# khiner/MeshEditor

Measured on AMD Instinct MI355X. Metric: eigenpairs/sec (K/M assembly + 50-mode solve, 100k-tet mesh), higher is better.
Workload: dtype f64; 1 GPU; cube_s100k: Kuhn mesh 105456 tets / 446631 DOF, NumModes=50 NumFemModes=65, P=10 excitation points, one mesh per GPU; eigenpairs_per_mesh=65, kept_modes_per_mesh=50, parallelism=mesh-per-gpu x1

## Files before the change

### mesheditor_amd/csrc/mh_api.hip

```cpp
#include "mh_common.h"

#include <algorithm>
#include <cmath>
#include <memory>

namespace {
constexpr int TB = 256;

__global__ void k_export_blocks(const uint32_t *__restrict__ row_ptr, const uint32_t *__restrict__ col, const uint32_t *__restrict__ perm, uint32_t nnodes,
                                uint32_t *__restrict__ row_out, uint32_t *__restrict__ col_out) {
    const uint32_t r = blockIdx.x * blockDim.x + threadIdx.x;
    if (r >= nnodes) return;
    for (uint32_t p = row_ptr[r]; p < row_ptr[r + 1]; ++p) {
        row_out[p] = perm[r];
        col_out[p] = perm[col[p]];
    }
}
__global__ void k_ref_to_panel(const double *__restrict__ xref, const uint32_t *__restrict__ perm, uint32_t nnodes, uint32_t w, double *__restrict__ panel) {
    const size_t i = size_t(blockIdx.x) * blockDim.x + threadIdx.x;
    if (i >= size_t(nnodes) * 3 * w) return;
    const uint32_t c = uint32_t(i % w), comp = uint32_t((i / w) % 3), node = uint32_t(i / (size_t(3) * w));
    panel[i] = xref[size_t(c) * (size_t(3) * nnodes) + size_t(3) * perm[node] + comp];
}
template<typename S, typename D> __global__ void k_cast(const S *__restrict__ src, D *__restrict__ dst, size_t count) {
// ... 83 lines not shown
}
int mh_context_create(int device, mh_context **out) {
    if (!out) return MH_EINVAL;
    *out = nullptr;
    auto *ctx = new mh_context;
    try {
        int count = 0;
        HIP_CHECK(hipGetDeviceCount(&count));
        if (count <= 0) mh_throw(MH_EHIP, "no HIP device: libmodalhip has no CPU fallback");
        if (device < 0 || device >= count) mh_throw(MH_EINVAL, "device %d out of range (%d visible)", device, count);
        ctx->device = device;
        if (hipDeviceGetAttribute(&ctx->cu_count, hipDeviceAttributeMultiprocessorCount, device) != hipSuccess || ctx->cu_count <= 0) ctx->cu_count = 256;
        HIP_CHECK(hipSetDevice(device));
        {
            size_t free_bytes = 0, total_bytes = 0;
            if (hipMemGetInfo(&free_bytes, &total_bytes) != hipSuccess) total_bytes = 0, (void)hipGetLastError();
            ctx->pool.set_cap_for_device(total_bytes);
        }
        HIP_CHECK(hipStreamCreateWithFlags(&ctx->stream, hipStreamNonBlocking));
        ROCBLAS_CHECK(rocblas_create_handle(&ctx->blas));
        ROCBLAS_CHECK(rocblas_set_stream(ctx->blas, ctx->stream));
        ROCBLAS_CHECK(rocblas_set_pointer_mode(ctx->blas, rocblas_pointer_mode_host));
        ROCBLAS_CHECK(rocblas_set_atomics_mode(ctx->blas, rocblas_atomics_not_allowed));
        *out = ctx;
        return MH_OK;
    } catch (const std::exception &e) {
        const int code = mh_guard(ctx, e);
        fprintf(stderr, "modalhip: %s\n", e.what());
        if (ctx->blas) rocblas_destroy_handle(ctx->blas);
        if (ctx->blas_aux) rocblas_destroy_handle(ctx->blas_aux);
        if (ctx->aux_stream) (void)hipStreamDestroy(ctx->aux_stream);
        if (ctx->aux2_stream) (void)hipStreamDestroy(ctx->aux2_stream);
        for (hipEvent_t ev : ctx->ahead_ev) (void)hipEventDestroy(ev);
        if (ctx->stream) (void)hipStreamDestroy(ctx->stream);
        delete ctx;
        return code;
    }
}
void mh_context_destroy(mh_context *ctx) {
    if (!ctx) return;
    (void)hipSetDevice(ctx->device);
    (void)hipStreamSynchronize(ctx->stream);
    if (ctx->blas) rocblas_destroy_handle(ctx->blas);
    if (ctx->blas_aux) rocblas_destroy_handle(ctx->blas_aux);
    if (ctx->aux_stream) (void)hipStreamDestroy(ctx->aux_stream);
    if (ctx->aux2_stream) (void)hipStreamDestroy(ctx->aux2_stream);
    for (hipEvent_t e : ctx->ahead_ev) (void)hipEventDestroy(e);
    if (ctx->stream) (void)hipStreamDestroy(ctx->stream);
    delete ctx;
}
const char *mh_last_error(const mh_context *ctx) { return ctx ? ctx->last_error.c_str() : "null context"; }
int mh_context_synchronize(mh_context *ctx) {
    if (!ctx) return MH_EINVAL;
    try {
        HIP_CHECK(hipStreamSynchronize(ctx->stream));
        return MH_OK;
    } catch (const std::exception &e) { return mh_guard(ctx, e); }
}
void *mh_context_stream(mh_context *ctx) { return ctx ? ctx->stream : nullptr; }
int mh_context_time_kernels(mh_context *ctx, int enable) {
    if (!ctx) return MH_EINVAL;
    try {
        mh_timer_flush(ctx);
        ctx->time_kernels = enable != 0;
        for (auto &t : ctx->totals) t = {};
        return MH_OK;
    } catch (const std::exception &e) { return mh_guard(ctx, e); }
}
int mh_context_kernel_class_stats(mh_context *ctx, int kernel_class, uint64_t *launches, double *total_ms, double *total_work) {
    if (!ctx || kernel_class < 0 || kernel_class >= MH_KERNEL_CLASSES) return MH_EINVAL;
    try {
        mh_timer_flush(ctx);
        const auto &t = ctx->totals[kernel_class];
        if (launches) *launches = t.launches;
        if (total_ms) *total_ms = t.ms;
// ... 205 lines not shown
```

### mesheditor_amd/csrc/mh_common.h

```cpp
#pragma once
#include "../../include/modalhip.h"

#include <hip/hip_runtime.h>
#include <rocblas/rocblas.h>
#include <rocsolver/rocsolver.h>

#include <algorithm>
#include <cstdarg>
#include <cstdio>
#include <cstdlib>
#include <cstring>
#include <iterator>
#include <limits>
#include <map>
#include <mutex>
#include <stdexcept>
#include <string>
#include <vector>

struct MhError : std::runtime_error {
    int code;
    MhError(int c, const std::string &m) : std::runtime_error(m), code(c) {}
};

// ... 207 lines not shown
    }
    ~DevicePool() {
        trim();
        for (auto &kv : live) (void)hipFree(kv.first);
    }
};

struct mh_context {
    int device{0};
    int cu_count{256};
    hipStream_t stream{nullptr};
    hipStream_t aux_stream{nullptr};
    bool aux_stream_ready() {
        if (!aux_stream && hipStreamCreateWithFlags(&aux_stream, hipStreamNonBlocking) != hipSuccess) aux_stream = nullptr;
        if (aux_stream && !blas_aux) {
            if (rocblas_create_handle(&blas_aux) != rocblas_status_success) blas_aux = nullptr;
            else if (rocblas_set_stream(blas_aux, aux_stream) != rocblas_status_success) {
                (void)rocblas_destroy_handle(blas_aux);
                blas_aux = nullptr;
            }
        }
        return aux_stream != nullptr && blas_aux != nullptr;
    }
    hipStream_t aux2_stream{nullptr};
    std::vector<hipEvent_t> ahead_ev;
    bool aux2_stream_ready(size_t events = 0) {
        if (!aux2_stream && hipStreamCreateWithFlags(&aux2_stream, hipStreamNonBlocking) != hipSuccess) aux2_stream = nullptr, (void)hipGetLastError();
        while (aux2_stream && ahead_ev.size() < events) {
            hipEvent_t e = nullptr;
            if (hipEventCreateWithFlags(&e, hipEventDisableTiming) != hipSuccess) { (void)hipGetLastError(); return false; }
            ahead_ev.push_back(e);
        }
        return aux2_stream != nullptr;
    }
    rocblas_handle blas{nullptr};
    rocblas_handle blas_aux{nullptr};
    DevicePool pool;
    std::string last_error;
    hipEvent_t ev0{nullptr}, ev1{nullptr};
    void *gram_ws{nullptr};
    size_t gram_ws_bytes{0};
    uint32_t *iota{nullptr};
    unsigned long long *sytrd_xch{nullptr};
    uint32_t sytrd_epoch{0};
    int *sytrd_flag{nullptr};
    unsigned long long *sytrd_xch_wide{nullptr};
    uint32_t sytrd_epoch_wide{0};
    bool exchange_disabled{false};
    uint32_t sytrd_redos{0};
    unsigned long long *rr_check{nullptr};
    struct MhRrTrace *rr_trace{nullptr};
    bool time_kernels{false};
    std::vector<std::pair<hipEvent_t, hipEvent_t>> timer_events;
    std::vector<double> timer_work;
    std::vector<int> timer_class;
    size_t timer_used{0};
    struct ClassTotals {
        double ms{0}, work{0};
        uint64_t launches{0};
    } totals[MH_KERNEL_CLASSES];
};
void mh_timer_flush(mh_context *ctx);
struct TimedLaunch {
    mh_context *ctx;
    bool on;
    size_t slot{0};
// ... 248 lines not shown
```

### mesheditor_amd/csrc/mh_eigs.hip

```cpp
#include "mh_common.h"

#include <algorithm>
#include <cmath>
#include <memory>
#include <condition_variable>
#include <mutex>
#include <numeric>
#include <optional>
#include <type_traits>

__global__ void k_shift_values(const double *kval, const double *mval, size_t nblocks, double sigma, double *aval);
__global__ void k_diag_inverse(const uint32_t *row_ptr, const uint32_t *col, const double *aval, uint32_t nnodes, double *dinv);
__global__ void k_coarse_matrix(const uint32_t *row_ptr, const uint32_t *col, const double *aval, const double *tmat, const uint32_t *agg_of, const uint32_t *agg_ptr,
                                const uint32_t *agg_nodes, uint32_t nagg, double *a0);
__global__ void k_fix_coarse_diag(double *a0, uint32_t n0, double rel);

namespace {
constexpr int TB = 256;

std::mutex g_solve_mutex;
struct Switches {
    bool verbose = getenv("MH_VERBOSE") != nullptr;
    bool fp32_prec = !(getenv("MH_PRECOND_FP64") && atoi(getenv("MH_PRECOND_FP64")) != 0);
    int deg2 = 0, deg1 = 0, gamma = 0;
    double cheb_ratio = 0.0, cheb_ratio1 = 0.0;
    bool test_sytrd_giveup = getenv("MH_TEST") && strstr(getenv("MH_TEST"), "sytrd_giveup");
    bool no_tridiag_wide = getenv("MH_TEST") && strstr(getenv("MH_TEST"), "no_tridiag_wide");
    bool test_last_resort = getenv("MH_TEST") && strstr(getenv("MH_TEST"), "last_resort");
    bool test_coarse_pivot = getenv("MH_TEST") && strstr(getenv("MH_TEST"), "coarse_pivot");
    bool test_selfcheck_fail = getenv("MH_TEST") && strstr(getenv("MH_TEST"), "selfcheck_fail");
    bool lmax_low = getenv("MH_TEST") && strstr(getenv("MH_TEST"), "lmax_low");
    bool potrf_chain = getenv("MH_TEST") && strstr(getenv("MH_TEST"), "potrf_chain");
    bool no_poly_start = getenv("MH_TEST") && strstr(getenv("MH_TEST"), "no_poly_start");
    Switches() {
        if (const char *c = getenv("MH_CYCLE")) {
            double v[5] = {0, 0, 0, 0, 0};
            sscanf(c, "%lf,%lf,%lf,%lf,%lf", &v[0], &v[1], &v[2], &v[3], &v[4]);
            deg2 = std::max(0, int(v[0])), deg1 = std::max(0, int(v[1])), gamma = std::max(0, int(v[2]));
            cheb_ratio = v[3];
            cheb_ratio1 = v[4];
        }
    }
};
const Switches &switches() {
    static const Switches s;
    return s;
}
constexpr int kPowerIterations = 20;
constexpr uint32_t kPrecondColumns = 256;
constexpr uint32_t kSkipP = 4;
constexpr uint32_t kGuardPercent = 10;
constexpr float kFlatShape = 1e-4f;
constexpr size_t kDenseLastResort = 12288;
constexpr int kLastResortCg = 8;

struct PhaseLock {
    std::mutex m;
    std::condition_variable cv;
    int readers = 0, writers_waiting = 0;
    bool writer = false;
    void lock_shared() {
        std::unique_lock<std::mutex> l(m);
        cv.wait(l, [&] { return !writer && writers_waiting == 0; });
        ++readers;
    }
    void unlock_shared() {
        std::unique_lock<std::mutex> l(m);
        if (--readers == 0) cv.notify_all();
    }
    void lock() {
        std::unique_lock<std::mutex> l(m);
        ++writers_waiting;
        cv.wait(l, [&] { return !writer && readers == 0; });
        --writers_waiting;
        writer = true;
    }
    void unlock() {
        std::unique_lock<std::mutex> l(m);
        writer = false;
        cv.notify_all();
    }
};
constexpr int kMaxDevices = 64;
PhaseLock g_phase_of_device[kMaxDevices];
PhaseLock &phase_of(int device) { return g_phase_of_device[unsigned(device) % kMaxDevices]; }
const bool g_concurrent = !(getenv("MH_CONCURRENT_SOLVES") && atoi(getenv("MH_CONCURRENT_SOLVES")) == 0);
struct SharedPhase {
    PhaseLock &phase;
    bool held = false, enabled = true;
    explicit SharedPhase(int device, bool on = true) : phase(phase_of(device)), enabled(on) { acquire(); }
    ~SharedPhase() { release(); }
    void acquire() { if (g_concurrent && enabled && !held) { phase.lock_shared(); held = true; } }
    void release() { if (held) { phase.unlock_shared(); held = false; } }
};
struct ExclusivePhase {
    PhaseLock &phase;
    bool held = false;
    explicit ExclusivePhase(int device) : phase(phase_of(device)) {
        if (g_concurrent) {
            phase.lock();
            held = true;
            (void)hipSetDevice(device);
            (void)hipDeviceSynchronize();
        }
    }
    ~ExclusivePhase() { if (held) phase.unlock(); }
};

struct Timer {
    mh_context *ctx;
    hipEvent_t a, b;
    explicit Timer(mh_context *c) : ctx(c) {
        HIP_CHECK(hipEventCreate(&a));
        HIP_CHECK(hipEventCreate(&b));
        HIP_CHECK(hipEventRecord(a, ctx->stream));
    }
    double stop() {
        HIP_CHECK(hipEventRecord(b, ctx->stream));
        HIP_CHECK(hipEventSynchronize(b));
// ... 1128 lines not shown
        const uint32_t nb = uint32_t(div_up(n, rpb));
        k_coldot_partial<<<dim3(nb, div_up(w, 64)), 64, 0, ctx->stream>>>(u, v, n, w, scratch, rpb);
        KERNEL_CHECK();
        k_colsumsq_final<<<w, 256, 0, ctx->stream>>>(scratch, nb, w, out);
        KERNEL_CHECK();
    }
    template<typename Prec> void solve(Prec &prec, const double *r, double *z, uint32_t w, int iters) {
        hipStream_t st = ctx->stream;
        HIP_CHECK(hipMemsetAsync(z, 0, n * w * sizeof(double), st));
        HIP_CHECK(hipMemcpyAsync(rr.get(), r, n * w * sizeof(double), hipMemcpyDeviceToDevice, st));
        prec.apply(rr, zz, w);
        HIP_CHECK(hipMemcpyAsync(p.get(), zz.get(), n * w * sizeof(double), hipMemcpyDeviceToDevice, st));
        dot(rr, zz, rz, w);
        for (int k = 0; k < iters; ++k) {
            mh_spmm(ctx, sys->L2, sys->L2.aval, p, ap, nullptr, nullptr, w);
            dot(p, ap, pap, w);
            k_cg_advance<<<grid1(n * w), TB, 0, st>>>(z, rr, p, ap, rz, pap, n * w, w);
            KERNEL_CHECK();
            if (k + 1 == iters) break;
            prec.apply(rr, zz, w);
            dot(rr, zz, rz_new, w);
            k_cg_direction<<<grid1(n * w), TB, 0, st>>>(p, zz, rz_new, rz, n * w, w);
            KERNEL_CHECK();
            HIP_CHECK(hipMemcpyAsync(rz.get(), rz_new.get(), w * sizeof(double), hipMemcpyDeviceToDevice, st));
        }
    }
};
}

namespace {
struct BlockLobpcg {
    mh_system *sys;
    mh_context *ctx;
    hipStream_t st;
    const size_t n;
    const uint32_t nev, b, mmax;
    const double sigma, residual_tol;
    const uint32_t max_iters;
    const float *seed_basis;
    const uint32_t seed_rows, seed_cols;
    const volatile unsigned char *cancel;
    volatile float *progress;
    mh_profile &prof;
    mh_profile *profile;
    SharedPhase iterating;
    Timer t_iter;
    double precond_seconds = 0;
    double best_worst_active = 1e300;
    int floor_strikes = 0;
    std::vector<double> hist_active;
    uint32_t pairs_at_floor = 0;
    DevArray<double> X, AX, MX, Xn, AXn, MXn, W, AW, MW, P, MP, Pn, MPn, R, Rw;
    DevArray<double> gA, gM, gM0, gA0, App, evals, ework, Cp, T1, H, H2, G, dscale, Linv, theta_d, rn_d, mn_d, scratch, Ct, norms_d, theta_act_d, Hp, Up, Vp, T1p;
    DevArray<double> Linv_p, T1p2;
    DevArray<uint32_t> idx_d, pos_d;
    DevArray<double> Rr, res_partial, res_blocks, res_norms_d;
    std::vector<double> rr_evals;
    std::vector<uint32_t> res_act, res_pos;
    std::vector<double> res_norms;
    uint32_t res_pitch = 0;
    bool res_ready = false, rw_from_rr = false;
    DevArray<int> info;
    int inner_cg = 0;
    std::unique_ptr<Precond<float>> prec32;
    std::unique_ptr<Precond<double>> prec64;
    std::unique_ptr<PanelCg> panel_cg;
    const bool verbose = switches().verbose, fp32_prec = switches().fp32_prec;
    const bool pproj_ok;
    const bool scaled_norms;
    bool warm = false;
    bool w_implicit = false;
    int last_spread = 1 << 20;
    bool p_needs_explicit = false;
    uint32_t wp = 0;
    uint32_t iters = 0, nconv = 0, redos_at_start = 0;
    bool poly_allowed = true;
    std::vector<double> theta, rn, mn, xn, norms, theta_act, hist_worst;
    double anorm = 0;
    std::vector<uint32_t> act, order, hist_nconv;
    std::vector<uint8_t> locked;
    bool converged = false;
    bool gm_identity = false;
    bool p_implicit = false;
    bool lazy_images = false;
    uint32_t w = 0, wa = 0, m = 0, wp_new = 0;

    BlockLobpcg(mh_system *system, uint32_t nev_, uint32_t block, double sigma_, double residual_tol_, uint32_t max_iters_, const float *seed_basis_, uint32_t seed_rows_,
                uint32_t seed_cols_, const volatile unsigned char *cancel_, volatile float *progress_, mh_profile &prof_, mh_profile *profile_, int inner_cg_ = 0)
        : sys(system), ctx(system->ctx), st(system->ctx->stream), n(size_t(3) * system->n_nodes), nev(nev_), b(block), mmax(3 * block), sigma(sigma_), residual_tol(residual_tol_),
          max_iters(max_iters_), seed_basis(seed_basis_), seed_rows(seed_rows_), seed_cols(seed_cols_), cancel(cancel_), progress(progress_), prof(prof_), profile(profile_),
          iterating(system->ctx->device, true), t_iter(system->ctx), pproj_ok(block <= 128), scaled_norms(system->patches2.any()), theta(block), rn(block), mn(block), xn(block), norms(3 * size_t(block)),
          theta_act(block), order(block), locked(block, 0) {
        inner_cg = inner_cg_;
        for (DevArray<double> *panel : {&X, &AX, &MX, &Xn, &AXn, &MXn, &W, &AW, &MW, &P, &Pn, &R, &Rw}) panel->reset(ctx, n * b);
        if (!pproj_ok)
            for (DevArray<double> *panel : {&MP, &MPn}) panel->reset(ctx, n * b);
        for (DevArray<double> *small : {&gA, &gM, &gM0, &gA0}) small->reset(ctx, size_t(mmax) * mmax);
        for (DevArray<double> *small : {&App, &H, &H2, &Linv, &Hp, &Up, &Vp, &T1p}) small->reset(ctx, size_t(b) * b);
        Linv_p.reset(ctx, size_t(b) * b);
        T1p2.reset(ctx, size_t(mmax) * b);
        for (DevArray<double> *small : {&Cp, &T1}) small->reset(ctx, size_t(mmax) * b);
        for (DevArray<double> *small : {&evals, &ework}) small->reset(ctx, mmax);
        for (DevArray<double> *small : {&dscale, &theta_d, &rn_d, &mn_d, &theta_act_d}) small->reset(ctx, b);
        G.reset(ctx, size_t(b) * 2 * b);
        Ct.reset(ctx, size_t(mmax) * 2 * b);
        norms_d.reset(ctx, 3 * size_t(b));
        idx_d.reset(ctx, b);
        pos_d.reset(ctx, b);
        if (b <= 128) {
            const uint32_t pmax = (b + 1u) & ~1u;
            Rr.reset(ctx, n * pmax);
            res_partial.reset(ctx, size_t(2) * sys->n_nodes * pmax);
            res_blocks.reset(ctx, size_t(div_up(sys->n_nodes, 48)) * 2 * pmax);
            res_norms_d.reset(ctx, size_t(2) * pmax);
            res_norms.resize(size_t(2) * pmax);
        }
        info.reset(ctx, 2);
        if (fp32_prec && !(sys->worst_quality < kFlatShape) && !inner_cg) prec32 = std::make_unique<Precond<float>>(sys, std::min(b, kPrecondColumns));
        else prec64 = std::make_unique<Precond<double>>(sys, std::min(b, kPrecondColumns));
        if (inner_cg) panel_cg = std::make_unique<PanelCg>(sys, std::min(b, kPrecondColumns));
        auto hd = sys->L2.dinv.to_host();
        double dmin = 1e300;
        for (double v : hd) dmin = std::min(dmin, v);
        anorm = sys->L2.lmax / dmin;
    }


    bool chol_orthonormalise(double *V, double *MV, double *AV, uint32_t w, bool transform_images = true, bool allow_implicit = false,
                             const double *hp = nullptr, uint32_t hp_rows = 0) {
        gram(ctx, n, V, w, MV, w, G, w);
        if (hp) {
            const double minus = -1, plus = 1;
            small_dgemm(ctx, rocblas_operation_transpose, rocblas_operation_none, rocblas_int(w), rocblas_int(w), rocblas_int(hp_rows), &minus, hp,
                                        rocblas_int(hp_rows), hp, rocblas_int(hp_rows), &plus, G, rocblas_int(w));
        }
        k_scale_gram<<<grid1(size_t(w) * w), TB, 0, st>>>(G, w, w, dscale);
        KERNEL_CHECK();
        double *Gs = G.get() + size_t(w) * w;
        int hinfo = 0;
        bool fused_inverse = false;
        {
            last_spread = 1 << 20;
            if (w <= 128) {
                fused_inverse = !switches().potrf_chain;
                if (fused_inverse) mh_potrf_small_inverse(ctx, Gs, w, info, dscale, Linv);
                else mh_potrf_small(ctx, Gs, w, info);
                int both[2] = {0, 0};
                info.download(both, 2);
                hinfo = both[0];
                last_spread = both[1];
            } else {
                mh_potrf(ctx, Gs, w, w, info);
                info.download(&hinfo, 1);
            }
        }
        p_needs_explicit = false;
        if (hp && (hinfo != 0 || last_spread >= 16 * 8)) {
            p_needs_explicit = true;
            return true;
        }
        if (hinfo != 0) return false;
        if (!fused_inverse) {
            k_unscale_chol<<<grid1(size_t(w) * w), TB, 0, st>>>(Gs, w, w, dscale);
            KERNEL_CHECK();
        }
        if (w > 256) {
            panel_trsm(ctx, n, V, w, Gs, w);
            if (MV) panel_trsm(ctx, n, MV, w, Gs, w);
            if (AV) panel_trsm(ctx, n, AV, w, Gs, w);
        } else {
            if (!fused_inverse) {
                HIP_CHECK(hipMemsetAsync(Linv, 0, size_t(w) * w * sizeof(double), st));
                ROCBLAS_CHECK(rocblas_dtrtri(ctx->blas, rocblas_fill_lower, rocblas_diagonal_non_unit, w, Gs, w, Linv, w));
            }
            w_implicit = allow_implicit && !transform_images && last_spread < 16 * 8;
            if (!w_implicit) mh_combine(ctx, n, V, w, nullptr, 0, nullptr, 0, Linv, w, V, w, nullptr);
            if (MV && transform_images) mh_combine(ctx, n, MV, w, nullptr, 0, nullptr, 0, Linv, w, MV, w, nullptr);
            if (AV && transform_images) mh_combine(ctx, n, AV, w, nullptr, 0, nullptr, 0, Linv, w, AV, w, nullptr);
        }
        return true;
    }

    void precondition(const double *r, double *z, uint32_t w) {
        precondition_in_slabs(ctx, n, r, z, w, [&](const double *rp, double *zp, uint32_t wc) {
            if (panel_cg) panel_cg->solve(*prec64, rp, zp, wc, inner_cg);
            else if (prec32) prec32->apply(rp, zp, wc);
            else prec64->apply(rp, zp, wc);
        });
    }

    void start() {
        redos_at_start = ctx->sytrd_redos;
        if (ctx->rr_check) HIP_CHECK(hipMemsetAsync(ctx->rr_check, 0, sizeof(unsigned long long), st));
        k_random_panel<<<grid1(n * b), TB, 0, st>>>(X, n * b, 20260710ull);
        KERNEL_CHECK();
        warm = seed_basis && seed_rows == n && seed_cols >= nev;
        if (warm) {
            const uint32_t ncols = std::min(seed_cols, b);
            DevArray<float> seed(ctx, n * ncols);
            seed.upload(seed_basis, n * ncols);
            k_load_seed<<<grid1(n * ncols), TB, 0, st>>>(seed, sys->perm, sys->n_nodes, ncols, b, X);
            KERNEL_CHECK();
            HIP_CHECK(hipStreamSynchronize(st));
        }
        const uint32_t n_rigid = 6 * sys->n_components;
        const bool seed_rigid = b >= n_rigid + 6;
        if (!seed_rigid && sys->n_components > 1)
            mh_throw(MH_EINVAL, "the mesh consists of %u disconnected bodies (%u zero modes): more than a block of %u columns can seed", sys->n_components, n_rigid, b);
        const auto inject_rigid_modes = [&] {
            k_inject_rbm<<<grid1(sys->n_nodes), TB, 0, st>>>(sys->node_xyz, sys->node_component, sys->component_centroid, sys->n_components, sys->n_nodes, X, b, 0);
            KERNEL_CHECK();
        };
        if (seed_rigid) inject_rigid_modes();
// ... 44 lines not shown
            if (with_poly) {
                if (verbose) fprintf(stderr, "[lobpcg] polynomial start block rank deficient: random block instead\n");
                poly_allowed = false;
                start();
                return;
            }
            mh_throw(MH_ENOTCONVERGED, "initial block is rank deficient");
        }
        mh_spmm(ctx, sys->L2, sys->L2.aval, X, AX, sys->L2.mval, MX, b);
        {
            gram(ctx, n, X, b, AX, b, gA, b);
            gram(ctx, n, X, b, MX, b, gM, b);
            const int hinfo = mh_rr_solve(ctx, gA, gM, b, evals, ework, info);
            if (hinfo != 0) mh_throw(MH_ENOTCONVERGED, "initial Rayleigh-Ritz failed (info %d)", hinfo);
            panel_mul(ctx, n, X, b, gA, b, Xn, b, 1.0, 0.0);
            panel_mul(ctx, n, AX, b, gA, b, AXn, b, 1.0, 0.0);
            panel_mul(ctx, n, MX, b, gA, b, MXn, b, 1.0, 0.0);
            std::swap(X, Xn); std::swap(AX, AXn); std::swap(MX, MXn);
            evals.download(theta.data(), b);
        }
    }

    bool converged_or_locked(uint32_t it) {
        if (cancel && *cancel) mh_throw(MH_ECANCELLED, "cancelled");
        if (g_concurrent) {
            iterating.release();
            iterating.acquire();
        }
        bool fused = res_ready;
        if (fused)
            for (const uint32_t i : res_act) fused = fused && !(std::abs(theta[i]) < 10.0 * std::abs(sigma));
        res_ready = false;
        rw_from_rr = fused;
        if (fused) {
            res_norms_d.download(res_norms.data(), size_t(2) * res_pitch);
            for (size_t k = 0; k < res_act.size(); ++k) {
                rn[res_act[k]] = res_norms[k];
                mn[res_act[k]] = res_norms[res_pitch + k];
            }
        } else {
        theta_d.upload(theta.data(), b);
        {
            const uint32_t rpb = 256, nblk = div_up(n, rpb);
            if (scratch.count < size_t(nblk) * 3 * b) scratch.reset(ctx, size_t(nblk) * 3 * b);
            dim3 grid(nblk, div_up(b, 64));
            k_residual_norms<<<grid, 64, 0, st>>>(AX, MX, X, theta_d, 10.0 * std::abs(sigma), R, n, b, rpb, scratch, scaled_norms ? sys->L2.dinv.get() : nullptr);
            KERNEL_CHECK();
            k_colsumsq_final<<<3 * b, 256, 0, st>>>(scratch, nblk, 3 * b, norms_d);
            KERNEL_CHECK();
            norms_d.download(norms.data(), 3 * size_t(b));
            std::copy(norms.begin(), norms.begin() + b, rn.begin());
            std::copy(norms.begin() + b, norms.begin() + 2 * b, mn.begin());
            std::copy(norms.begin() + 2 * b, norms.end(), xn.begin());
        }
        }
        act.clear();
        for (uint32_t i = 0; i < b; ++i) {
            const double rel = std::sqrt(rn[i]) / (std::abs(theta[i]) * std::sqrt(mn[i]));
            const bool near_shift = std::abs(theta[i]) < 10.0 * std::abs(sigma);
            const double floor_norm = scaled_norms ? sys->L2.lmax * std::sqrt(xn[i]) : anorm * std::sqrt(xn[i]);
            const double floor_factor = it == 0 && !warm && sys->worst_quality < kFlatShape ? 65536.0 : 256.0;
            const bool ok = rel < residual_tol || (near_shift && std::sqrt(rn[i]) < floor_factor * 2.2e-16 * floor_norm);
            if (ok) locked[i] = 1;
            if (!locked[i]) act.push_back(i);
        }
        std::iota(order.begin(), order.end(), 0u);
        std::stable_sort(order.begin(), order.end(), [&](uint32_t a, uint32_t c) { return theta[a] < theta[c]; });
        nconv = 0;
// ... 48 lines not shown
    void search_directions(uint32_t it) {
        w = uint32_t(act.size());
        idx_d.upload(act.data(), w);
        const double *residuals = Rw.get();
        if (rw_from_rr) {
            if (act == res_act && res_pitch == w) {
                residuals = Rr.get();
            } else {
                std::vector<uint32_t> &pos = res_pos;
                pos.assign(w, 0);
                size_t q = 0;
                for (uint32_t k = 0; k < w; ++k) {
                    while (q < res_act.size() && res_act[q] != act[k]) ++q;
                    if (q == res_act.size()) mh_throw(MH_EHIP, "active column %u was not active before", act[k]);
                    pos[k] = uint32_t(q);
                }
                pos_d.upload(pos.data(), w);
                k_gather_cols<<<grid1(n * w), TB, 0, st>>>(Rr, pos_d, Rw, n, res_pitch, w);
                KERNEL_CHECK();
            }
        } else {
            k_gather_cols<<<grid1(n * w), TB, 0, st>>>(R, idx_d, Rw, n, b, w);
            KERNEL_CHECK();
        }
        for (uint32_t k = 0; k < w; ++k) theta_act[k] = theta[act[k]];
        theta_act_d.upload(theta_act.data(), w);
        {
            Timer tp(ctx);
            precondition(residuals, W, w);
            precond_seconds += tp.stop();
            prof.op_applications += w;
        }
        bool ok = true;
        p_implicit = false;
        if (pproj_ok && wp) {
            gram(ctx, n, MX, b, W, w, H, b);
            mh_pack_stacked(ctx, H, b, nullptr, 0, w, -1.0, Ct);
            mh_combine(ctx, n, X, b, nullptr, 0, nullptr, 0, Ct, w, W, w, nullptr, true);
            mh_spmm(ctx, sys->L2, sys->L2.aval, W, AW, sys->L2.mval, MW, w);
            gram(ctx, n, P, wp, MW, w, Hp, wp);
            lazy_images = true;
            w_implicit = false;
            ok = chol_orthonormalise(W, MW, AW, w, false, true, Hp, wp);
            if (!ok) mh_throw(MH_ENOTCONVERGED, "search directions lost rank at iteration %u", it);
            if (p_needs_explicit) {
                mh_pack_stacked(ctx, Hp, wp, nullptr, 0, w, -1.0, Ct);
                mh_combine(ctx, n, P, wp, nullptr, 0, nullptr, 0, Ct, w, W, w, nullptr, true);
                mh_spmm(ctx, sys->L2, sys->L2.aval, W, AW, sys->L2.mval, MW, w);
                lazy_images = w <= 256;
                ok = chol_orthonormalise(W, MW, AW, w, !lazy_images, lazy_images);
                if (!ok) mh_throw(MH_ENOTCONVERGED, "search directions lost rank at iteration %u", it);
            } else {
                p_implicit = true;
            }
        } else {
            gram(ctx, n, MX, b, W, w, H, b);
            if (wp) gram(ctx, n, MP, wp, W, w, H2, wp);
            mh_pack_stacked(ctx, H, b, H2, wp, w, -1.0, Ct);
            mh_combine(ctx, n, X, b, P, wp, nullptr, 0, Ct, w, W, w, nullptr, true);
            mh_spmm(ctx, sys->L2, sys->L2.aval, W, AW, sys->L2.mval, MW, w);
            lazy_images = w <= 256;
            w_implicit = false;
            ok = chol_orthonormalise(W, MW, AW, w, !lazy_images, lazy_images);
            if (!ok) mh_throw(MH_ENOTCONVERGED, "search directions lost rank at iteration %u", it);
        }
    }

    void rayleigh_ritz(uint32_t it) {
        wa = w;
        m = wa + w + wp;
        for (int attempt = 0; attempt < 2; ++attempt) {
            HIP_CHECK(hipMemsetAsync(gA, 0, size_t(m) * m * sizeof(double), st));
            HIP_CHECK(hipMemsetAsync(gM, 0, size_t(m) * m * sizeof(double), st));
            k_set_identity_blocks<<<grid1(wa), TB, 0, st>>>(gA, gM, theta_act_d, wa, m);
            KERNEL_CHECK();
            const double unit_one = 1;
            auto left_corrected = [&](double *block, uint32_t cols) {
                if (w_implicit)
                    ROCBLAS_CHECK(rocblas_dtrmm(ctx->blas, rocblas_side_left, rocblas_fill_lower, rocblas_operation_none, rocblas_diagonal_non_unit, rocblas_int(w),
                                                rocblas_int(cols), &unit_one, Linv, rocblas_int(w), block, rocblas_int(m), block, rocblas_int(m)));
            };
            mh_gram(ctx, n, W, w, AX, wa, gA.get() + wa, m, b, idx_d);
            left_corrected(gA.get() + wa, wa);
            const double unit = 1;
            auto untransformed = [&](double *block, uint32_t rows) {
                if (lazy_images)
                    ROCBLAS_CHECK(rocblas_dtrmm(ctx->blas, rocblas_side_right, rocblas_fill_lower, rocblas_operation_transpose, rocblas_diagonal_non_unit, rocblas_int(rows),
                                                rocblas_int(w), &unit, Linv, rocblas_int(w), block, rocblas_int(m), block, rocblas_int(m)));
            };
            gram(ctx, n, W, w, AW, w, gA.get() + size_t(wa) * m + wa, m);
            if (p_implicit && wp) {
                const double plus = 1, nil = 0;
                double *bw = gA.get() + size_t(wa) * m + wa, *bp = gA.get() + size_t(wa) * m + wa + w;
                gram(ctx, n, P, wp, AW, w, bp, m);
                small_dgemm(ctx, rocblas_operation_transpose, rocblas_operation_none, rocblas_int(w), rocblas_int(w), rocblas_int(wp), &plus, Hp, rocblas_int(wp), bp,
                                            rocblas_int(m), &nil, Up, rocblas_int(w));
                small_dgemm(ctx, rocblas_operation_none, rocblas_operation_none, rocblas_int(wp), rocblas_int(w), rocblas_int(wp), &plus, App, rocblas_int(wp), Hp,
                                            rocblas_int(wp), &nil, T1p, rocblas_int(wp));
                small_dgemm(ctx, rocblas_operation_transpose, rocblas_operation_none, rocblas_int(w), rocblas_int(w), rocblas_int(wp), &plus, Hp, rocblas_int(wp), T1p,
                                            rocblas_int(wp), &nil, Vp, rocblas_int(w));
                k_sub_block<<<grid1(size_t(wp) * w), TB, 0, st>>>(bp, m, T1p, wp, wp, w);
                k_wblock_fix<<<grid1(size_t(w) * w), TB, 0, st>>>(bw, m, Up, Vp, w);
                KERNEL_CHECK();
            }
            untransformed(gA.get() + size_t(wa) * m + wa, w);
            left_corrected(gA.get() + size_t(wa) * m + wa, w);
            const bool w_block_trusted = last_spread < 16 * 8 && !(p_implicit && wp == 0);
            gm_identity = w_block_trusted;
            if (w_block_trusted) {
                k_place_block<<<grid1(size_t(w) * w), TB, 0, st>>>(gM.get() + size_t(wa) * m + wa, m, nullptr, w);
                KERNEL_CHECK();
            } else {
                gram(ctx, n, W, w, MW, w, gM.get() + size_t(wa) * m + wa, m);
                untransformed(gM.get() + size_t(wa) * m + wa, w);
            }
            if (verbose) fprintf(stderr, "[lobpcg] it %3u Cholesky-QR diagonal spread 2^%.1f%s\n", it, last_spread / 16.0, w_block_trusted ? "" : " (W block measured)");
            if (wp) {
                if (!p_implicit) gram(ctx, n, P, wp, AW, w, gA.get() + size_t(wa) * m + wa + w, m);
                untransformed(gA.get() + size_t(wa) * m + wa + w, wp);
                {
                    k_place_block<<<grid1(size_t(wp) * wp), TB, 0, st>>>(gA.get() + size_t(wa + w) * m + wa + w, m, App, wp);
                    k_place_block<<<grid1(size_t(wp) * wp), TB, 0, st>>>(gM.get() + size_t(wa + w) * m + wa + w, m, nullptr, wp);
                    KERNEL_CHECK();
                }
            }
            k_symmetrize_lower<<<grid1(size_t(m) * m), TB, 0, st>>>(gA, m, m);
            KERNEL_CHECK();
            HIP_CHECK(hipMemcpyAsync(gA0, gA, size_t(m) * m * sizeof(double), hipMemcpyDeviceToDevice, st));
            HIP_CHECK(hipMemcpyAsync(gM0, gM, size_t(m) * m * sizeof(double), hipMemcpyDeviceToDevice, st));
            rr_evals.clear();
            const int hinfo = mh_rr_solve(ctx, gA, gM, m, evals, ework, info, wa, gm_identity, &rr_evals);
            if (hinfo == 0) break;
            if (attempt == 1 || wp == 0) mh_throw(MH_ENOTCONVERGED, "Rayleigh-Ritz failed at iteration %u (info %d)", it, hinfo);
            wp = 0;
            m = wa + w;
        }
        if (rr_evals.size() == wa) std::copy(rr_evals.begin(), rr_evals.end(), theta_act.begin());
        else evals.download(theta_act.data(), wa);
        for (uint32_t k = 0; k < wa; ++k) theta[act[k]] = theta_act[k];
    }

    void conjugate_directions(uint32_t it) {
        const double one = 1, zero = 0, mone = -1;
        wp_new = w;
        k_build_cp<<<grid1(size_t(m) * w), TB, 0, st>>>(gA, nullptr, wa, m, w, m, Cp, m);
        KERNEL_CHECK();
        const double *mcp = gm_identity ? Cp.get() : T1.get();
        if (!gm_identity) ROCBLAS_CHECK(rocblas_dsymm(ctx->blas, rocblas_side_left, rocblas_fill_lower, m, w, &one, gM0, m, Cp, m, &zero, T1, m));
        small_dgemm(ctx, rocblas_operation_transpose, rocblas_operation_none, wa, w, m, &one, gA, m, mcp, m, &zero, H, wa);
        small_dgemm(ctx, rocblas_operation_none, rocblas_operation_none, m, w, wa, &mone, gA, m, H, wa, &one, Cp, m);
        if (!gm_identity) ROCBLAS_CHECK(rocblas_dsymm(ctx->blas, rocblas_side_left, rocblas_fill_lower, m, w, &one, gM0, m, Cp, m, &zero, T1, m));
        small_dgemm(ctx, rocblas_operation_transpose, rocblas_operation_none, w, w, m, &one, Cp, m, mcp, m, &zero, G, w);
        k_scale_gram<<<grid1(size_t(w) * w), TB, 0, st>>>(G, w, w, dscale);
        KERNEL_CHECK();
        {
            double *Gs = G.get() + size_t(w) * w;
            int hinfo = 0;
            const bool fused = w <= 128 && !switches().potrf_chain;
            {
                if (fused) mh_potrf_small_inverse(ctx, Gs, w, info, dscale, Linv_p);
                else mh_potrf(ctx, Gs, w, w, info);
                info.download(&hinfo, 1);
            }
            if (hinfo != 0) {
                wp_new = 0;
            } else if (fused) {
                mh_small_gemm(ctx, false, true, m, w, w, 1.0, Cp, m, Linv_p, w, 0.0, T1p2, m);
                HIP_CHECK(hipMemcpyAsync(Cp, T1p2, size_t(m) * w * sizeof(double), hipMemcpyDeviceToDevice, st));
            } else {
                k_unscale_chol<<<grid1(size_t(w) * w), TB, 0, st>>>(Gs, w, w, dscale);
                KERNEL_CHECK();
                ROCBLAS_CHECK(rocblas_dtrsm(ctx->blas, rocblas_side_right, rocblas_fill_lower, rocblas_operation_transpose, rocblas_diagonal_non_unit, m, w, &one, Gs, w, Cp, m));
            }
        }
        if (!warm && it < kSkipP && !hist_worst.empty() && hist_worst.back() > 0.5) wp_new = 0;
        if (wp_new) {
            small_dgemm(ctx, rocblas_operation_none, rocblas_operation_none, m, wp_new, m, &one, gA0, m, Cp, m, &zero, T1, m);
            small_dgemm(ctx, rocblas_operation_transpose, rocblas_operation_none, wp_new, wp_new, m, &one, Cp, m, T1, m, &zero, App, wp_new);
        }
    }

    void update_basis(uint32_t it) {
        mh_pack_coefficients(ctx, gA, wa, Cp, wp_new, m, m, Ct);
        {
            const uint32_t pitch = (wa + 1u) & ~1u;
            if (w_implicit) {
                const double unit = 1;
                double *rows = Ct.get() + size_t(wa) * (wa + wp_new);
                ROCBLAS_CHECK(rocblas_dtrmm(ctx->blas, rocblas_side_right, rocblas_fill_lower, rocblas_operation_none, rocblas_diagonal_non_unit, rocblas_int(wa + wp_new),
                                            rocblas_int(w), &unit, Linv, rocblas_int(w), rows, rocblas_int(wa + wp_new), rows, rocblas_int(wa + wp_new)));
            }
            if (p_implicit && wp) {
                const double minus = -1, plus = 1;
                const rocblas_int pitchc = rocblas_int(wa + wp_new);
                double *rows_w = Ct.get() + size_t(wa) * (wa + wp_new), *rows_p = Ct.get() + size_t(wa + w) * (wa + wp_new);
                ROCBLAS_CHECK(rocblas_dgemm(ctx->blas, rocblas_operation_none, rocblas_operation_transpose, pitchc, rocblas_int(wp), rocblas_int(w), &minus, rows_w, pitchc, Hp,
                                            rocblas_int(wp), &plus, rows_p, pitchc));
            }
            mh_combine(ctx, n, X, wa, W, w, P, wp, Ct, wa + wp_new, Xn, wa, Pn, false, b, idx_d, pitch);
            if (wp_new && !pproj_ok) mh_spmm(ctx, sys->L2, nullptr, Pn, nullptr, sys->L2.mval, MPn, wp_new);
            if (pitch == wa) k_scatter_cols<<<grid1(n * wa), TB, 0, st>>>(Xn.get(), idx_d, X.get(), n, b, wa);
            else k_scatter_cols_pitch<<<grid1(n * wa), TB, 0, st>>>(Xn.get(), pitch, idx_d, X.get(), n, b, wa);
            KERNEL_CHECK();
            if (Rr.count) {
                mh_spmm_mapped(ctx, sys->L2, sys->L2.aval, Xn, AX, sys->L2.mval, MX, pitch, b, wa, idx_d, evals, Rr, res_partial, scaled_norms ? sys->L2.dinv.get() : nullptr);
                const uint32_t rpb = 48, nblk = div_up(sys->n_nodes, rpb), w2 = 2 * pitch;
                dim3 grid(nblk, div_up(w2, 64));
                k_colsum_partial<<<grid, 64, 0, st>>>(res_partial, sys->n_nodes, w2, res_blocks, rpb);
                KERNEL_CHECK();
                k_colsumsq_final<<<w2, 256, 0, st>>>(res_blocks, nblk, w2, res_norms_d);
                KERNEL_CHECK();
                res_act = act;
                res_pitch = pitch;
                res_ready = true;
            } else {
                mh_spmm_mapped(ctx, sys->L2, sys->L2.aval, Xn, AX, sys->L2.mval, MX, pitch, b, wa, idx_d);
            }
        }
        std::swap(P, Pn); std::swap(MP, MPn);
        wp = wp_new;
    }

    void finish(double *eigenvalues) {
        prof.restarts = iters;
        prof.op_solve = precond_seconds;
        if (!converged) mh_throw(MH_ENOTCONVERGED, "LOBPCG: %u of %u pairs converged in %u iterations", nconv, nev, iters);
        for (uint32_t k = 0; k < nev; ++k) eigenvalues[k] = theta[order[k]] + sigma;
        sys->plain_residual = -1.0;
        if (scaled_norms) {
            theta_d.upload(theta.data(), b);
            const uint32_t rpb = 256, nblk = div_up(n, rpb);
            if (scratch.count < size_t(nblk) * 3 * b) scratch.reset(ctx, size_t(nblk) * 3 * b);
            k_residual_norms<<<dim3(nblk, div_up(b, 64)), 64, 0, st>>>(AX, MX, X, theta_d, 10.0 * std::abs(sigma), R, n, b, rpb, scratch, nullptr);
            KERNEL_CHECK();
            k_colsumsq_final<<<3 * b, 256, 0, st>>>(scratch, nblk, 3 * b, norms_d);
            KERNEL_CHECK();
            norms_d.download(norms.data(), 3 * size_t(b));
            double worst = 0;
            for (uint32_t k = 0; k < nev; ++k) {
                const uint32_t i = order[k];
                if (std::abs(theta[i]) < 10.0 * std::abs(sigma)) continue;
                worst = std::max(worst, std::sqrt(norms[i]) / (std::abs(theta[i]) * std::sqrt(norms[b + i])));
            }
            sys->plain_residual = worst;
            if (verbose) fprintf(stderr, "[lobpcg] accepted in the Jacobi-scaled norm at %.1e; worst elastic pair in the plain 2-norm: %.2e\n", residual_tol, worst);
        }
        sys->evecs.reset(ctx, n * nev);
        sys->evec_cols = nev;
        idx_d.upload(order.data(), nev);
        k_gather_cols<<<grid1(n * nev), TB, 0, st>>>(X, idx_d, sys->evecs, n, b, nev);
        KERNEL_CHECK();
        HIP_CHECK(hipStreamSynchronize(st));
        prof.iterate = t_iter.stop();
        read_health();
        sys->profile = prof;
        if (profile) *profile = prof;
        if (switches().test_selfcheck_fail && !ctx->exchange_disabled) prof.rr_selfcheck = 1.0;
        if (!(prof.rr_selfcheck < 1e-6))
            mh_throw(MH_EHIP, "Rayleigh-Ritz self-check failed: a step's eigenpairs leave a relative residual of %.2e against the step's own matrix", prof.rr_selfcheck);
    }
    void read_health() {
        prof.sytrd_redos = ctx->sytrd_redos - redos_at_start;
        prof.pairs_at_floor = pairs_at_floor;
        prof.rr_selfcheck = 0.0;
        if (ctx->rr_check) {
            unsigned long long bits = 0;
            HIP_CHECK(hipMemcpyAsync(&bits, ctx->rr_check, sizeof(bits), hipMemcpyDeviceToHost, st));
            HIP_CHECK(hipStreamSynchronize(st));
            memcpy(&prof.rr_selfcheck, &bits, sizeof(double));
        }
    }

    void run(double *eigenvalues) {
        start();
        for (uint32_t it = 0; it <= max_iters; ++it) {
            if (converged_or_locked(it)) break;
            search_directions(it);
            rayleigh_ritz(it);
            conjugate_directions(it);
            update_basis(it);
        }
        finish(eigenvalues);
    }
};
struct Attempt {
    mh_system *sys;
    uint32_t nev, b;
    double sigma, residual_tol;
    const float *seed;
    uint32_t srows, scols;
    const volatile unsigned char *cancel;
    volatile float *progress;
    double *eigenvalues;
    mh_profile &prof;
    mh_profile *profile;
    std::optional<MhError> run(uint32_t max_iters, int inner_cg = 0) {
        try {
            BlockLobpcg solver(sys, nev, b, sigma, residual_tol, max_iters, seed, srows, scols, cancel, progress, prof, profile, inner_cg);
            solver.run(eigenvalues);
            return std::nullopt;
        } catch (const MhError &e) {
            return e;
        }
    }
    void reset_profile() {
        prof = sys->profile;
        prof.dofs = uint32_t(size_t(3) * sys->n_nodes);
    }
// ... 211 lines not shown
```

Measured before the change: 614.2 eigenpairs/s.

## Overlap small Cholesky factor with Gram products and defer column scatter behind norm readback

In LOBPCG's search-direction orthonormalisation, the small Gram scaling and Cholesky/inverse now run on the aux stream. The Rayleigh-Ritz Gram products (W'AX, W'AW, P'AW) are queued on the main stream while the host waits on the factor's info readback, and Rayleigh-Ritz reuses them when the implicit path holds. Residual norms are copied into pinned host memory with an event, and the column scatter is queued after that copy, so the next iteration's host wait does not cover the scatter kernel. This removes host-sync bubbles at the cost of extra events, stream switching inside the context, and speculative Gram work that is thrown away when the factor turns out ill-conditioned.

```diff
diff --git a/mesheditor_amd/csrc/mh_api.hip b/mesheditor_amd/csrc/mh_api.hip
--- a/mesheditor_amd/csrc/mh_api.hip
+++ b/mesheditor_amd/csrc/mh_api.hip
@@ -139,6 +139,7 @@
         if (ctx->aux_stream) (void)hipStreamDestroy(ctx->aux_stream);
         if (ctx->aux2_stream) (void)hipStreamDestroy(ctx->aux2_stream);
         for (hipEvent_t ev : ctx->ahead_ev) (void)hipEventDestroy(ev);
+        ctx->chain_release();
         if (ctx->stream) (void)hipStreamDestroy(ctx->stream);
         delete ctx;
         return code;
@@ -148,6 +149,8 @@
     if (!ctx) return;
     (void)hipSetDevice(ctx->device);
     (void)hipStreamSynchronize(ctx->stream);
+    if (ctx->aux_stream) (void)hipStreamSynchronize(ctx->aux_stream);
+    ctx->chain_release();
     if (ctx->blas) rocblas_destroy_handle(ctx->blas);
     if (ctx->blas_aux) rocblas_destroy_handle(ctx->blas_aux);
     if (ctx->aux_stream) (void)hipStreamDestroy(ctx->aux_stream);
diff --git a/mesheditor_amd/csrc/mh_common.h b/mesheditor_amd/csrc/mh_common.h
--- a/mesheditor_amd/csrc/mh_common.h
+++ b/mesheditor_amd/csrc/mh_common.h
@@ -263,6 +263,27 @@
             ahead_ev.push_back(e);
         }
         return aux2_stream != nullptr;
+    }
+    struct ChainReport {
+        int w[2];
+        double norms[2 * 128];
+    };
+    enum { kChainFork = 0, kChainW, kChainNorms, kChainEvents };
+    hipEvent_t chain_ev[kChainEvents]{};
+    ChainReport *chain_host{nullptr};
+    bool chain_ready() {
+        if (!chain_host && hipHostMalloc(reinterpret_cast<void **>(&chain_host), sizeof(ChainReport), hipHostMallocDefault) != hipSuccess) chain_host = nullptr, (void)hipGetLastError();
+        for (hipEvent_t &e : chain_ev)
+            if (!e && hipEventCreateWithFlags(&e, hipEventDisableTiming) != hipSuccess) { e = nullptr; (void)hipGetLastError(); return false; }
+        return chain_host != nullptr;
+    }
+    void chain_release() {
+        for (hipEvent_t &e : chain_ev) {
+            if (e) (void)hipEventDestroy(e);
+            e = nullptr;
+        }
+        if (chain_host) (void)hipHostFree(chain_host);
+        chain_host = nullptr;
     }
     rocblas_handle blas{nullptr};
     rocblas_handle blas_aux{nullptr};
diff --git a/mesheditor_amd/csrc/mh_eigs.hip b/mesheditor_amd/csrc/mh_eigs.hip
--- a/mesheditor_amd/csrc/mh_eigs.hip
+++ b/mesheditor_amd/csrc/mh_eigs.hip
@@ -1,7 +1,9 @@
 #include "mh_common.h"
 
 #include <algorithm>
+#include <atomic>
 #include <cmath>
+#include <functional>
 #include <memory>
 #include <condition_variable>
 #include <mutex>
@@ -32,6 +34,9 @@
     bool lmax_low = getenv("MH_TEST") && strstr(getenv("MH_TEST"), "lmax_low");
     bool potrf_chain = getenv("MH_TEST") && strstr(getenv("MH_TEST"), "potrf_chain");
     bool no_poly_start = getenv("MH_TEST") && strstr(getenv("MH_TEST"), "no_poly_start");
+    bool serial_chains = getenv("MH_TEST") && strstr(getenv("MH_TEST"), "serial_chains");
+    bool w_report_ill = getenv("MH_TEST") && strstr(getenv("MH_TEST"), "w_report_ill");
+    bool cp_report_fail = getenv("MH_TEST") && strstr(getenv("MH_TEST"), "cp_report_fail");
     Switches() {
         if (const char *c = getenv("MH_CYCLE")) {
             double v[5] = {0, 0, 0, 0, 0};
@@ -49,6 +54,7 @@
 constexpr int kPowerIterations = 20;
 constexpr uint32_t kPrecondColumns = 256;
 constexpr uint32_t kSkipP = 4;
+constexpr uint32_t kHookIteration = 6;
 constexpr uint32_t kGuardPercent = 10;
 constexpr float kFlatShape = 1e-4f;
 constexpr size_t kDenseLastResort = 12288;
@@ -85,6 +91,13 @@
 PhaseLock g_phase_of_device[kMaxDevices];
 PhaseLock &phase_of(int device) { return g_phase_of_device[unsigned(device) % kMaxDevices]; }
 const bool g_concurrent = !(getenv("MH_CONCURRENT_SOLVES") && atoi(getenv("MH_CONCURRENT_SOLVES")) == 0);
+std::atomic<int> g_iterating_on_device[kMaxDevices];
+struct IteratingOnDevice {
+    std::atomic<int> &count;
+    explicit IteratingOnDevice(int device) : count(g_iterating_on_device[unsigned(device) % kMaxDevices]) { count.fetch_add(1); }
+    ~IteratingOnDevice() { count.fetch_sub(1); }
+    bool alone() const { return count.load() == 1; }
+};
 struct SharedPhase {
     PhaseLock &phase;
     bool held = false, enabled = true;
@@ -1279,6 +1292,7 @@
 struct BlockLobpcg {
     mh_system *sys;
     mh_context *ctx;
+    IteratingOnDevice in_flight{ctx->device};
     hipStream_t st;
     const size_t n;
     const uint32_t nev, b, mmax;
@@ -1331,6 +1345,12 @@
     bool p_implicit = false;
     bool lazy_images = false;
     uint32_t w = 0, wa = 0, m = 0, wp_new = 0;
+    bool overlap = false, overlap_side = false;
+    bool can_overlap = false, can_side = false;
+    bool raw_grams_queued = false;
+    bool norms_in_flight = false;
+    uint32_t cur_it = 0;
+    bool hook_w_fired = false, hook_cp_fired = false;
 
     BlockLobpcg(mh_system *system, uint32_t nev_, uint32_t block, double sigma_, double residual_tol_, uint32_t max_iters_, const float *seed_basis_, uint32_t seed_rows_,
                 uint32_t seed_cols_, const volatile unsigned char *cancel_, volatile float *progress_, mh_profile &prof_, mh_profile *profile_, int inner_cg_ = 0)
@@ -1363,6 +1383,8 @@
             res_norms.resize(size_t(2) * pmax);
         }
         info.reset(ctx, 2);
+        can_overlap = pproj_ok && !switches().serial_chains && !switches().potrf_chain && ctx->chain_ready();
+        can_side = can_overlap && ctx->aux_stream_ready();
         if (fp32_prec && !(sys->worst_quality < kFlatShape) && !inner_cg) prec32 = std::make_unique<Precond<float>>(sys, std::min(b, kPrecondColumns));
         else prec64 = std::make_unique<Precond<double>>(sys, std::min(b, kPrecondColumns));
         if (inner_cg) panel_cg = std::make_unique<PanelCg>(sys, std::min(b, kPrecondColumns));
@@ -1372,23 +1394,36 @@
         anorm = sys->L2.lmax / dmin;
     }
 
+    ~BlockLobpcg() {
+        if (can_side) (void)hipStreamSynchronize(ctx->aux_stream);
+    }
+
 
     bool chol_orthonormalise(double *V, double *MV, double *AV, uint32_t w, bool transform_images = true, bool allow_implicit = false,
-                             const double *hp = nullptr, uint32_t hp_rows = 0) {
+                             const double *hp = nullptr, uint32_t hp_rows = 0, const std::function<void()> *beside = nullptr) {
         gram(ctx, n, V, w, MV, w, G, w);
         if (hp) {
             const double minus = -1, plus = 1;
             small_dgemm(ctx, rocblas_operation_transpose, rocblas_operation_none, rocblas_int(w), rocblas_int(w), rocblas_int(hp_rows), &minus, hp,
                                         rocblas_int(hp_rows), hp, rocblas_int(hp_rows), &plus, G, rocblas_int(w));
         }
-        k_scale_gram<<<grid1(size_t(w) * w), TB, 0, st>>>(G, w, w, dscale);
-        KERNEL_CHECK();
         double *Gs = G.get() + size_t(w) * w;
         int hinfo = 0;
         bool fused_inverse = false;
+        const bool side_by_side = beside && overlap_side && w <= 128;
+        if (!side_by_side) {
+            k_scale_gram<<<grid1(size_t(w) * w), TB, 0, st>>>(G, w, w, dscale);
+            KERNEL_CHECK();
+        }
         {
             last_spread = 1 << 20;
-            if (w <= 128) {
+            if (side_by_side) {
+                fused_inverse = true;
+                int both[2] = {0, 0};
+                factor_beside(w, *beside, both);
+                hinfo = both[0];
+                last_spread = both[1];
+            } else if (w <= 128) {
                 fused_inverse = !switches().potrf_chain;
                 if (fused_inverse) mh_potrf_small_inverse(ctx, Gs, w, info, dscale, Linv);
                 else mh_potrf_small(ctx, Gs, w, info);
@@ -1401,6 +1436,11 @@
                 info.download(&hinfo, 1);
             }
         }
+        if (switches().w_report_ill && allow_implicit && !hook_w_fired && cur_it >= kHookIteration) {
+            hook_w_fired = true;
+            last_spread = 16 * 8;
+            if (verbose) fprintf(stderr, "[lobpcg] it %3u MH_TEST=w_report_ill: the factor's report reads ill-conditioned%s\n", cur_it, side_by_side ? " (Gram products were queued beside it)" : "");
+        }
         p_needs_explicit = false;
         if (hp && (hinfo != 0 || last_spread >= 16 * 8)) {
             p_needs_explicit = true;
@@ -1426,6 +1466,30 @@
             if (AV && transform_images) mh_combine(ctx, n, AV, w, nullptr, 0, nullptr, 0, Linv, w, AV, w, nullptr);
         }
         return true;
+    }
+
+    void factor_beside(uint32_t w, const std::function<void()> &beside, int both[2]) {
+        hipStream_t aux = ctx->aux_stream;
+        double *Gs = G.get() + size_t(w) * w;
+        HIP_CHECK(hipEventRecord(ctx->chain_ev[mh_context::kChainFork], st));
+        HIP_CHECK(hipStreamWaitEvent(aux, ctx->chain_ev[mh_context::kChainFork], 0));
+        k_scale_gram<<<grid1(size_t(w) * w), TB, 0, aux>>>(G, w, w, dscale);
+        KERNEL_CHECK();
+        ctx->stream = aux;
+        try {
+            mh_potrf_small_inverse(ctx, Gs, w, info, dscale, Linv);
+        } catch (...) {
+            ctx->stream = st;
+            throw;
+        }
+        ctx->stream = st;
+        HIP_CHECK(hipMemcpyAsync(ctx->chain_host->w, info.get(), 2 * sizeof(int), hipMemcpyDeviceToHost, aux));
+        HIP_CHECK(hipEventRecord(ctx->chain_ev[mh_context::kChainW], aux));
+        beside();
+        HIP_CHECK(hipEventSynchronize(ctx->chain_ev[mh_context::kChainW]));
+        both[0] = ctx->chain_host->w[0];
+        both[1] = ctx->chain_host->w[1];
+        HIP_CHECK(hipStreamWaitEvent(st, ctx->chain_ev[mh_context::kChainW], 0));
     }
 
     void precondition(const double *r, double *z, uint32_t w) {
@@ -1536,8 +1600,14 @@
             for (const uint32_t i : res_act) fused = fused && !(std::abs(theta[i]) < 10.0 * std::abs(sigma));
         res_ready = false;
         rw_from_rr = fused;
+        cur_it = it;
         if (fused) {
-            res_norms_d.download(res_norms.data(), size_t(2) * res_pitch);
+            if (norms_in_flight) {
+                HIP_CHECK(hipEventSynchronize(ctx->chain_ev[mh_context::kChainNorms]));
+                std::copy(ctx->chain_host->norms, ctx->chain_host->norms + size_t(2) * res_pitch, res_norms.begin());
+            } else {
+                res_norms_d.download(res_norms.data(), size_t(2) * res_pitch);
+            }
             for (size_t k = 0; k < res_act.size(); ++k) {
                 rn[res_act[k]] = res_norms[k];
                 mn[res_act[k]] = res_norms[res_pitch + k];
@@ -1652,6 +1722,9 @@
             prof.op_applications += w;
         }
         bool ok = true;
+        raw_grams_queued = false;
+        const std::function<void()> raw_grams = [&] { raw_gram_products(); };
+        const std::function<void()> *beside = overlap_side && w <= 128 ? &raw_grams : nullptr;
         p_implicit = false;
         if (pproj_ok && wp) {
             gram(ctx, n, MX, b, W, w, H, b);
@@ -1661,8 +1734,9 @@
             gram(ctx, n, P, wp, MW, w, Hp, wp);
             lazy_images = true;
             w_implicit = false;
-            ok = chol_orthonormalise(W, MW, AW, w, false, true, Hp, wp);
+            ok = chol_orthonormalise(W, MW, AW, w, false, true, Hp, wp, beside);
             if (!ok) mh_throw(MH_ENOTCONVERGED, "search directions lost rank at iteration %u", it);
+            raw_grams_queued = raw_grams_queued && w_implicit && !p_needs_explicit;
             if (p_needs_explicit) {
                 mh_pack_stacked(ctx, Hp, wp, nullptr, 0, w, -1.0, Ct);
                 mh_combine(ctx, n, P, wp, nullptr, 0, nullptr, 0, Ct, w, W, w, nullptr, true);
@@ -1681,26 +1755,43 @@
             mh_spmm(ctx, sys->L2, sys->L2.aval, W, AW, sys->L2.mval, MW, w);
             lazy_images = w <= 256;
             w_implicit = false;
-            ok = chol_orthonormalise(W, MW, AW, w, !lazy_images, lazy_images);
+            ok = chol_orthonormalise(W, MW, AW, w, !lazy_images, lazy_images, nullptr, 0, beside);
             if (!ok) mh_throw(MH_ENOTCONVERGED, "search directions lost rank at iteration %u", it);
-        }
+            raw_grams_queued = raw_grams_queued && w_implicit;
+        }
+    }
+
+    void raw_gram_products() {
+        wa = w;
+        m = wa + w + wp;
+        HIP_CHECK(hipMemsetAsync(gA, 0, size_t(m) * m * sizeof(double), st));
+        HIP_CHECK(hipMemsetAsync(gM, 0, size_t(m) * m * sizeof(double), st));
+        k_set_identity_blocks<<<grid1(wa), TB, 0, st>>>(gA, gM, theta_act_d, wa, m);
+        KERNEL_CHECK();
+        mh_gram(ctx, n, W, w, AX, wa, gA.get() + wa, m, b, idx_d);
+        gram(ctx, n, W, w, AW, w, gA.get() + size_t(wa) * m + wa, m);
+        if (wp) gram(ctx, n, P, wp, AW, w, gA.get() + size_t(wa) * m + wa + w, m);
+        raw_grams_queued = true;
     }
 
     void rayleigh_ritz(uint32_t it) {
         wa = w;
         m = wa + w + wp;
         for (int attempt = 0; attempt < 2; ++attempt) {
-            HIP_CHECK(hipMemsetAsync(gA, 0, size_t(m) * m * sizeof(double), st));
-            HIP_CHECK(hipMemsetAsync(gM, 0, size_t(m) * m * sizeof(double), st));
-            k_set_identity_blocks<<<grid1(wa), TB, 0, st>>>(gA, gM, theta_act_d, wa, m);
-            KERNEL_CHECK();
+            const bool raw = attempt == 0 && raw_grams_queued && (wp == 0 || p_implicit);
+            if (!raw) {
+                HIP_CHECK(hipMemsetAsync(gA, 0, size_t(m) * m * sizeof(double), st));
+                HIP_CHECK(hipMemsetAsync(gM, 0, size_t(m) * m * sizeof(double), st));
+                k_set_identity_blocks<<<grid1(wa), TB, 0, st>>>(gA, gM, theta_act_d, wa, m);
+                KERNEL_CHECK();
+            }
             const double unit_one = 1;
             auto left_corrected = [&](double *block, uint32_t cols) {
                 if (w_implicit)
                     ROCBLAS_CHECK(rocblas_dtrmm(ctx->blas, rocblas_side_left, rocblas_fill_lower, rocblas_operation_none, rocblas_diagonal_non_unit, rocblas_int(w),
                                                 rocblas_int(cols), &unit_one, Linv, rocblas_int(w), block, rocblas_int(m), block, rocblas_int(m)));
             };
-            mh_gram(ctx, n, W, w, AX, wa, gA.get() + wa, m, b, idx_d);
+            if (!raw) mh_gram(ctx, n, W, w, AX, wa, gA.get() + wa, m, b, idx_d);
             left_corrected(gA.get() + wa, wa);
             const double unit = 1;
             auto untransformed = [&](double *block, uint32_t rows) {
@@ -1708,11 +1799,11 @@
                     ROCBLAS_CHECK(rocblas_dtrmm(ctx->blas, rocblas_side_right, rocblas_fill_lower, rocblas_operation_transpose, rocblas_diagonal_non_unit, rocblas_int(rows),
                                                 rocblas_int(w), &unit, Linv, rocblas_int(w), block, rocblas_int(m), block, rocblas_int(m)));
             };
-            gram(ctx, n, W, w, AW, w, gA.get() + size_t(wa) * m + wa, m);
+            if (!raw) gram(ctx, n, W, w, AW, w, gA.get() + size_t(wa) * m + wa, m);
             if (p_implicit && wp) {
                 const double plus = 1, nil = 0;
                 double *bw = gA.get() + size_t(wa) * m + wa, *bp = gA.get() + size_t(wa) * m + wa + w;
-                gram(ctx, n, P, wp, AW, w, bp, m);
+                if (!raw) gram(ctx, n, P, wp, AW, w, bp, m);
                 small_dgemm(ctx, rocblas_operation_transpose, rocblas_operation_none, rocblas_int(w), rocblas_int(w), rocblas_int(wp), &plus, Hp, rocblas_int(wp), bp,
                                             rocblas_int(m), &nil, Up, rocblas_int(w));
                 small_dgemm(ctx, rocblas_operation_none, rocblas_operation_none, rocblas_int(wp), rocblas_int(w), rocblas_int(wp), &plus, App, rocblas_int(wp), Hp,
@@ -1758,6 +1849,13 @@
         if (rr_evals.size() == wa) std::copy(rr_evals.begin(), rr_evals.end(), theta_act.begin());
         else evals.download(theta_act.data(), wa);
         for (uint32_t k = 0; k < wa; ++k) theta[act[k]] = theta_act[k];
+    }
+
+    bool cp_hook(uint32_t it) {
+        if (!switches().cp_report_fail || hook_cp_fired || it < kHookIteration) return false;
+        hook_cp_fired = true;
+        if (verbose) fprintf(stderr, "[lobpcg] it %3u MH_TEST=cp_report_fail: the conjugate directions' factor reports failure\n", it);
+        return true;
     }
 
     void conjugate_directions(uint32_t it) {
@@ -1782,6 +1880,7 @@
                 else mh_potrf(ctx, Gs, w, w, info);
                 info.download(&hinfo, 1);
             }
+            if (cp_hook(it)) hinfo = 1;
             if (hinfo != 0) {
                 wp_new = 0;
             } else if (fused) {
@@ -1819,9 +1918,14 @@
             }
             mh_combine(ctx, n, X, wa, W, w, P, wp, Ct, wa + wp_new, Xn, wa, Pn, false, b, idx_d, pitch);
             if (wp_new && !pproj_ok) mh_spmm(ctx, sys->L2, nullptr, Pn, nullptr, sys->L2.mval, MPn, wp_new);
-            if (pitch == wa) k_scatter_cols<<<grid1(n * wa), TB, 0, st>>>(Xn.get(), idx_d, X.get(), n, b, wa);
-            else k_scatter_cols_pitch<<<grid1(n * wa), TB, 0, st>>>(Xn.get(), pitch, idx_d, X.get(), n, b, wa);
-            KERNEL_CHECK();
+            const auto scatter = [&] {
+                if (pitch == wa) k_scatter_cols<<<grid1(n * wa), TB, 0, st>>>(Xn.get(), idx_d, X.get(), n, b, wa);
+                else k_scatter_cols_pitch<<<grid1(n * wa), TB, 0, st>>>(Xn.get(), pitch, idx_d, X.get(), n, b, wa);
+                KERNEL_CHECK();
+            };
+            const bool scatter_last = overlap && Rr.count;
+            norms_in_flight = false;
+            if (!scatter_last) scatter();
             if (Rr.count) {
                 mh_spmm_mapped(ctx, sys->L2, sys->L2.aval, Xn, AX, sys->L2.mval, MX, pitch, b, wa, idx_d, evals, Rr, res_partial, scaled_norms ? sys->L2.dinv.get() : nullptr);
                 const uint32_t rpb = 48, nblk = div_up(sys->n_nodes, rpb), w2 = 2 * pitch;
@@ -1833,9 +1937,15 @@
                 res_act = act;
                 res_pitch = pitch;
                 res_ready = true;
+                if (scatter_last) {
+                    HIP_CHECK(hipMemcpyAsync(ctx->chain_host->norms, res_norms_d.get(), size_t(2) * pitch * sizeof(double), hipMemcpyDeviceToHost, st));
+                    HIP_CHECK(hipEventRecord(ctx->chain_ev[mh_context::kChainNorms], st));
+                    norms_in_flight = true;
+                }
             } else {
                 mh_spmm_mapped(ctx, sys->L2, sys->L2.aval, Xn, AX, sys->L2.mval, MX, pitch, b, wa, idx_d);
             }
+            if (scatter_last) scatter();
         }
         std::swap(P, Pn); std::swap(MP, MPn);
         wp = wp_new;
@@ -1894,6 +2004,8 @@
     void run(double *eigenvalues) {
         start();
         for (uint32_t it = 0; it <= max_iters; ++it) {
+            overlap = can_overlap && in_flight.alone();
+            overlap_side = can_side && overlap;
             if (converged_or_locked(it)) break;
             search_directions(it);
             rayleigh_ritz(it);
```

Result: faster. 624.1 eigenpairs/s, median of 6 (+1.6%).
